# ilia-glushchenko/SimplePathTracer

Measured on AMD Instinct MI355X. Metric: Msamples/s (pixels×spp/s), RTIOW random-sphere scene, 1/2/4/8 MI355X, higher is better.
Workload: dtype f32

## Files before the change

### simplepathtracer_amd/csrc/spt_internal.h

```cpp
#pragma once
#include <hip/hip_runtime.h>
#include <stdint.h>

#include "spt_hip.h"

namespace spt {

struct RowMap {
    uint32_t y0, y1, strip, parts, part;
    uint32_t x0, width;
};

__host__ __device__ inline uint32_t row_of(const RowMap &m, uint32_t lr)
{
    uint32_t blk = lr / m.strip;
    return m.y0 + (blk * m.parts + m.part) * m.strip + (lr - blk * m.strip);
}

__host__ __device__ inline uint32_t rows_owned(const RowMap &m)
{
    if (m.y1 <= m.y0) return 0;
    uint32_t h = m.y1 - m.y0;
    uint32_t period = m.strip * m.parts;
    uint32_t full = h / period, rem = h % period;
// ... 43 lines not shown
inline FastDiv make_fastdiv(uint32_t d)
{
    FastDiv f{d, 0u, 0u};
    if (d <= 1u) return f;
    uint32_t l = 0;
    while ((1ull << l) < d) ++l;
    f.m = (uint32_t)(((1ull << (31 + l)) / d) + 1ull);
    f.s = l - 1u;
    return f;
}
__host__ __device__ inline uint32_t fast_div(uint32_t x, const FastDiv &f)
{
#ifdef __HIP_DEVICE_COMPILE__
    const uint32_t hi = __umulhi(x, f.m);
#else
    const uint32_t hi = (uint32_t)(((uint64_t)x * f.m) >> 32);
#endif
    return f.d <= 1u ? x : hi >> f.s;
}

__host__ __device__ inline uint32_t row_of_fast(const RowMap &m, uint32_t lr, const FastDiv &div_strip)
{
    const uint32_t blk = fast_div(lr, div_strip);
    return m.y0 + (blk * m.parts + m.part) * m.strip + (lr - blk * m.strip);
}

struct DealRule {
    uint64_t below;
    uint32_t q, rem;
};
constexpr DealRule make_deal_rule(uint32_t np)
{
    DealRule r{0ull, 0u, 0u};
    if (np == 0u || np > 64u) return r;
    r.q = 64u / np;
    r.rem = 64u - r.q * np;
    uint32_t start = 0;
    for (uint32_t k = 0; k < np; ++k) {
        if (start > 0u) r.below |= 1ull << (start - 1u);
        start += r.q + (k < r.rem ? 1u : 0u);
    }
    return r;
}
struct DealTable {
    DealRule e[65];
    constexpr DealTable() : e{}
    {
        for (uint32_t np = 0; np <= 64u; ++np) e[np] = make_deal_rule(np);
    }
};
static constexpr DealTable kDealTable{};
__host__ __device__ inline uint32_t deal_start(const DealRule &r, uint32_t rank)
{
    return rank * r.q + (rank < r.rem ? rank : r.rem);
}
__host__ __device__ inline uint32_t deal_count(const DealRule &r, uint32_t rank)
{
    return r.q + (rank < r.rem ? 1u : 0u);
}
__host__ __device__ inline void deal_lane(const DealRule &r, uint32_t lane, uint32_t &rank, uint32_t &tt)
{
#ifdef __HIP_DEVICE_COMPILE__
    rank = __builtin_amdgcn_mbcnt_hi((uint32_t)(r.below >> 32), __builtin_amdgcn_mbcnt_lo((uint32_t)r.below, 0u));
#else
    rank = (uint32_t)__builtin_popcountll(r.below & ((1ull << lane) - 1ull));
#endif
    tt = lane - deal_start(r, rank);
}

__host__ __device__ inline void ts_item(uint32_t q, uint32_t width, uint32_t rows, uint32_t S, const FastDiv &div_band,
                                        const FastDiv &div_tile, uint32_t &sl, uint32_t &lr, uint32_t &col)
{
    const uint32_t band = rows >= 8u ? fast_div(q, div_band) : 0u;
    const uint32_t h = rows - (band << 3) < 8u ? rows - (band << 3) : 8u;
    const uint32_t qb = q - band * 8u * width * S;
    const uint32_t ft = width >> 3, wr = width & 7u;
    const uint32_t ti = h * 8u * S;
    uint32_t e, wt, c0;
    if (h == 8u) {
        const uint32_t t = fast_div(qb, div_tile);
        if (t < ft) {
            e = qb - t * 64u * S;
            sl = e >> 6;
            const uint32_t pix = e & 63u;
            lr = (band << 3) + (pix >> 3);
            col = (t << 3) + (pix & 7u);
            return;
        }
        e = qb - ft * ti;
        wt = wr;
        c0 = ft << 3;
    } else {
        const uint32_t t = qb / ti;
        wt = t < ft ? 8u : wr;
        e = qb - (t < ft ? t : ft) * ti;
        c0 = (t < ft ? t : ft) << 3;
    }
    sl = e / (h * wt);
    const uint32_t pix = e - sl * h * wt;
    const uint32_t row = pix / wt;
    lr = (band << 3) + row;
    col = c0 + (pix - row * wt);
}

__host__ __device__ inline void ts_slot_base(uint32_t lr, uint32_t col, uint32_t width, uint32_t rows, uint32_t S,
                                             uint32_t &q0, uint32_t &step)
{
    const uint32_t band = lr >> 3;
    const uint32_t h = rows - (band << 3) < 8u ? rows - (band << 3) : 8u;
    const uint32_t ft = width >> 3, wr = width & 7u;
    const uint32_t t = col >> 3;
    const uint32_t tc = t < ft ? t : ft;
    const uint32_t wt = t < ft ? 8u : wr;
    q0 = band * 8u * width * S + tc * h * 8u * S + (lr - (band << 3)) * wt + (col - (tc << 3));
    step = h * wt;
}

constexpr uint32_t kCodeSmall = 0x33800000u;
constexpr uint32_t kCodeMax = 2u * (kCodeSmall - 1u);
constexpr uint32_t kCodeSat = 280;
__host__ __device__ inline bool code_layout_fits(uint64_t stride, uint32_t jmax)
// ... 271 lines not shown
```

### simplepathtracer_amd/csrc/spt_kernels.hip

```cpp
#include "spt_path.h"
#include "spt_decode.h"

#include <algorithm>
#include <mutex>

namespace spt {


#ifndef SPT_WAVES_PER_EU
#define SPT_WAVES_PER_EU 0
#endif
#ifndef SPT_NUM_SGPR
#define SPT_NUM_SGPR 96
#endif
#if SPT_WAVES_PER_EU
#define SPT_RENDER_ATTR __attribute__((amdgpu_waves_per_eu(SPT_WAVES_PER_EU, SPT_WAVES_PER_EU)))
#elif SPT_NUM_SGPR
#define SPT_CAP_WAVES (800 / (((SPT_NUM_SGPR - 2 + 15) / 16) * 16 + 16) > 8 ? 8 : 800 / (((SPT_NUM_SGPR - 2 + 15) / 16) * 16 + 16))
#define SPT_RENDER_ATTR __attribute__((amdgpu_num_sgpr(SPT_NUM_SGPR), amdgpu_waves_per_eu(SPT_CAP_WAVES)))
#else
#define SPT_RENDER_ATTR
#endif

#ifndef SPT_LDS_BLOCK
// ... 305 lines not shown
            if (v.y != 0u) {
                const f3 c = decode_sample(a, v.x);
                acc.x = acc.x + c.x;
                acc.y = acc.y + c.y;
                acc.z = acc.z + c.z;
                acc.w = acc.w + 1.f;
            }
        }
    } else {
        alias_accumulate(a, samples, p, W, rows, 0u, rows, S, acc);
    }
    if (!a.last) {
        a.acc[p] = acc;
        if (!a.preview) return;
    }
    const float scale = a.mode == 0 ? 1.f / (float)a.s_done : 1.f / acc.w;
    const float r = acc.x * scale, g = acc.y * scale, b = acc.z * scale;
    if (out_rgba) out_rgba[p] = make_float4(r, g, b, 0.f);
    if (out_rgb8) {
        const uint32_t x = map.x0 + col;
        const uint32_t y = row_of(map, lr);
        const size_t gi = (size_t)3 * ((size_t)(a.height - 1u - y) * a.width + x);
        out_rgb8[gi + 0] = gamma_byte(r);
        out_rgb8[gi + 1] = gamma_byte(g);
        out_rgb8[gi + 2] = gamma_byte(b);
    }
}

#ifndef SPT_SVC_WT
#define SPT_SVC_WT 1
#endif

__device__ __forceinline__ void svc_flush(uint32_t idx, uint32_t cnt, uint32_t lane)
{
    if (cnt == 0u) return;
    kargs_t &k = *kernarg_args();
    asm volatile("s_waitcnt vmcnt(0)" ::: "memory");
    if (!SPT_SVC_WT) {
        __builtin_amdgcn_fence(__ATOMIC_RELEASE, "agent");
        asm volatile("s_waitcnt vmcnt(0)" ::: "memory");
    }
    if (lane == 0) __hip_atomic_fetch_add((gu32 *)(k.svc_done + idx), cnt, __ATOMIC_RELAXED, __HIP_MEMORY_SCOPE_AGENT);
    if (k.svc_trace && lane == 0) atomicMax(k.svc_trace + 4u * idx + 2u, __builtin_amdgcn_s_memrealtime());
}

template <bool TREE, int LEAF, bool LDSN, uint32_t BLOCK, bool BATCH = false, bool GLANE = false, bool SVC = false>
__device__ __forceinline__ void render_body(const RenderArgs &a)
{
    static_assert(!SVC || (!GLANE && !BATCH && (LDSN || SPT_PRIM)),
                  "the render service runs the wave-walk kernel or the LDS lane walk");
    const uint32_t lane = __lane_id();
    const uint32_t rows = SVC ? 0u : a.npix / a.map.width;

    __shared__ uint32_t s_lds[BLOCK];
    __shared__ uint4 s_nodes[LDSN ? 2 * (SVC ? kLdsSvcNodeRecords : kLdsNodeRecords) : 1];
    constexpr bool LDS_BYTES = LDSN && SPT_LANE_WALK && SPT_LANE_BUDGET > 0;
    constexpr bool PRIM = SPT_PRIM && !LDSN && !GLANE;
    constexpr uint32_t PW = kParkWords + (SVC ? 1u : 0u);
    __shared__ uint32_t s_park[PRIM ? (BLOCK / 64u) * PW * 64u : 1];
    uint32_t *const park = s_park + (PRIM ? opaque_v((threadIdx.x >> 6) * PW * 64u + lane) : 0u);
    auto prow = [&](uint32_t r) -> int32_t { return (int32_t)r - (int32_t)lane; };
    __shared__ uint32_t s_rec[SVC ? (BLOCK / 64u) * kSvcRecWords : 1];
    uint32_t *const rec = s_rec + (SVC ? (threadIdx.x >> 6) * kSvcRecWords : 0u);
    if (SVC && lane < kSvcRecWords - kSvcSt) rec[kSvcSt + lane] = 0u;
    if (SVC && !LDSN && blockIdx.x == 0u && (threadIdx.x >> 6) == 0u) {
        svc_forward(lane);
        return;
    }
    uint32_t q_n = 0, q_pos = 0;
    if (LDSN) {
        const uint4 *src = (const uint4 *)a.scene.accel.nodes;
        const uint32_t n4 = 2u * (a.scene.accel.n_nodes + 1u);
        for (uint32_t k = threadIdx.x; k < n4; k += BLOCK) {
            uint4 v = src[k];
            if (LDS_BYTES && (k & 1u)) v.x <<= 5;
            s_nodes[k] = v;
        }
        __syncthreads();
        if (SVC && blockIdx.x == 0u && (threadIdx.x >> 6) == 0u) {
            svc_forward(lane);
            return;
        }
    }
    Path ps;
    ps.phase = PH_IDLE;
    ps.item = ps.bounce = ps.spec = 0;
    ps.st = 0;
    ps.o = ps.d = mk(0.f, 0.f, 0.f);
    ps.slot = 0;
    ps.job = 0;

    uint32_t blk_cur = 0, blk_end = 0;
    uint32_t pend = 0;
    uint32_t rect = 0;
    const uint32_t home = blockIdx.x % a.n_queues;
    uint32_t qi = 0;
    if (SVC)
        pend = svc_reserve(home, lane, 0u);
    else if (lane == 0)
        pend = claim_next(a, home, qi);
    bool exhausted = false;
    uint32_t acc_idx = 0, acc_cnt = 0;
    unsigned long long casts = 0, done = 0, dropped = 0;
    struct {
        unsigned long long iters = 0, cast = 0, shade = 0, refill = 0;
        unsigned long long p_iters = 0, p_nodes = 0, p_spheres = 0, p_branches = 0, p_cast = 0;
        unsigned long long s_rounds[3] = {0, 0, 0};
        unsigned long long t_iters = 0, t_live = 0;
    } dc;
    CastDiag dg;
    Hit hres;
    hres.idx = kMiss;
    hres.best = FLT_MAX;
    hres.t = 0.f;
    uint32_t li = 0, lleaf = kNoSlot, lleaf2 = kNoSlot;
    bool fresh = true;
#if SPT_DIAG
// ... 219 lines not shown
                }
                if (leave) break;
                continue;
            }
            if (exhausted && q_pos == q_n) break;
            continue;
        }
        SPT_STAMP(dc.refill);
#if SPT_DIAG
        const unsigned long long d_n0 = dg.nodes, d_s0 = dg.spheres, d_b0 = dg.branches, d_c0 = dc.cast;
#endif
        constexpr bool RES = SPT_LANE_BUDGET > 0 && (LDSN || GLANE);
        if (!RES) casts += (unsigned long long)__popcll(live);
        ++dc.iters;
        if (SPT_DIAG && exhausted) {
            dc.t_iters += 1;
            dc.t_live += (unsigned long long)__popcll(live);
        }
        const bool act = ps.phase != PH_IDLE;
        bool cdone = true;
        Hit h;
        if constexpr (RES) {
            if (SPT_DUP & 512) {
                Hit h2 = hres;
                h2.best = opaque_v(h2.best);
                uint32_t li2 = opaque_v(li), ll2 = lleaf, ll22 = lleaf2;
                const bool c2 = lane_cast<LEAF, LDS_BYTES>(a.scene.accel, opaque_v3(ps.o), opaque_v3(ps.d), act, dg,
                                    LDSN ? (const uint32_t *)s_nodes : (const uint32_t *)a.scene.accel.nodes, fresh,
                                    (uint32_t)SPT_LANE_BUDGET, h2, li2, ll2, ll22);
                sink_v(h2.idx);
                sink_v(h2.best);
                sink_v(li2);
                sink_v(c2 ? 1u : 0u);
            }
            cdone = lane_cast<LEAF, LDS_BYTES>(a.scene.accel, ps.o, ps.d, act, dg,
                                    LDSN ? (const uint32_t *)s_nodes : (const uint32_t *)a.scene.accel.nodes, fresh,
                                    (uint32_t)SPT_LANE_BUDGET, hres, li, lleaf, lleaf2);
            h = hres;
            casts += (unsigned long long)__popcll(__ballot(act && cdone));
        } else if constexpr (PRIM) {
            bool listed = false;
            if (prim_iter && kernarg_args()->prim.on) {
                if (SPT_DUP & 64) {
                    Hit h2;
                    prim_list_cast(a.scene.accel, opaque_v3(ps.o), opaque_v3(ps.d), act, pxy, h2, dg);
                    sink_v(h2.idx);
                    sink_v(h2.best);
                    sink_v(h2.t);
                }
                listed = prim_list_cast(a.scene.accel, ps.o, ps.d, act, pxy, h, dg);
            }
            if (!listed)
                h = find_closest<TREE, LEAF, LDSN>(a.scene.accel, ps.o, ps.d, act, dg, (const uint32_t *)s_nodes,
                                                   s_lds + (threadIdx.x & ~63u));
            if (SPT_DUP & 1) {
                const f3 o2 = opaque_v3(ps.o), d2 = opaque_v3(ps.d);
                Hit h2;
                bool l2 = false;
                if (prim_iter && kernarg_args()->prim.on) l2 = prim_list_cast(a.scene.accel, o2, d2, act, pxy, h2, dg);
                if (!l2) h2 = find_closest<TREE, LEAF, LDSN>(a.scene.accel, o2, d2, act, dg, (const uint32_t *)s_nodes);
                sink_v(h2.idx);
                sink_v(h2.best);
                sink_v(h2.t);
            }
        } else {
            h = (LDSN && SPT_LANE_WALK)
                    ? find_closest_lane<LEAF>(a.scene.accel, ps.o, ps.d, act, dg, (const uint32_t *)s_nodes)
                : GLANE
                    ? find_closest_lane<LEAF>(a.scene.accel, ps.o, ps.d, act, dg, (const uint32_t *)a.scene.accel.nodes)
                    : find_closest<TREE, LEAF, LDSN>(a.scene.accel, ps.o, ps.d, act, dg, (const uint32_t *)s_nodes);
        }
        SPT_STAMP(dc.cast);
#if SPT_DIAG
        if (prim_iter) {
            dc.p_iters += 1;
            dc.p_nodes += dg.nodes - d_n0;
            dc.p_spheres += dg.spheres - d_s0;
            dc.p_branches += dg.branches - d_b0;
            dc.p_cast += dc.cast - d_c0;
        }
#endif
        shade_step<true, SVC && SPT_SVC_WT>(a, ps, h, act && cdone, done, dropped, s_lds + (threadIdx.x & ~63u),
                                            SPT_DIAG ? dc.s_rounds : nullptr);
        fresh = cdone;
        if (SVC) {
            const bool fin = act && ps.phase == PH_IDLE;
            unsigned long long fm = __ballot(fin);
            while (fm != 0ull) {
                const uint32_t j = __builtin_amdgcn_readlane(ps.job, (int)__builtin_ctzll(fm));
                const unsigned long long m = __ballot(fin && ps.job == j);
                if (j != acc_idx) {
                    svc_flush(acc_idx, acc_cnt, lane);
                    acc_idx = j;
                    acc_cnt = 0;
                }
                acc_cnt += (uint32_t)__popcll(m);
                fm &= ~m;
            }
        }
        if (PRIM && prim_iter) {
            Path own;
            unpark_path<SVC>(park, 0, own);
            __builtin_amdgcn_wave_barrier();
            const unsigned long long lv = __ballot(ps.phase != PH_IDLE);
            if (ps.phase != PH_IDLE) park_path<SVC>(park, prow(lane_rank(lv)), ps);
            ps = own;
            q_n = (uint32_t)__popcll(lv);
            q_pos = 0;
        }
        SPT_STAMP(dc.shade);
    }

    if (SVC) {
        svc_flush(acc_idx, acc_cnt, lane);
        kargs_t &k = *kernarg_args();
        if (lane == 0) __hip_atomic_fetch_add((gu32 *)(k.svc_ctl + kSvcLive), 0xFFFFFFFFu, __ATOMIC_RELAXED, __HIP_MEMORY_SCOPE_AGENT);
    }
#pragma unroll
    for (int o = 32; o > 0; o >>= 1) {
        done += __shfl_xor(done, o);
        dropped += __shfl_xor(dropped, o);
    }
    if (lane == 0) {
        if (casts) atomicAdd(&a.counters[0], casts);
        if (done) atomicAdd(&a.counters[1], done);
        if (dropped) atomicAdd(&a.counters[2], dropped);
    }
#if SPT_DIAG
    if (lane == 0) {
        atomicAdd(&a.counters[4], dc.iters);
        atomicAdd(&a.counters[5], dg.leaves);
        atomicAdd(&a.counters[6], dg.nodes);
        atomicAdd(&a.counters[7], dc.cast);
        atomicAdd(&a.counters[8], dc.shade);
        atomicAdd(&a.counters[9], dc.refill);
// ... 353 lines not shown
```

### simplepathtracer_amd/csrc/spt_path.h

```cpp
#pragma once
#include "spt_device.h"
#include "spt_internal.h"

#include <float.h>

#ifndef SPT_GROUP
#define SPT_GROUP 4
#endif

#ifndef SPT_DIAG
#define SPT_DIAG 0
#endif
#ifndef SPT_LEAF_SPLIT
#define SPT_LEAF_SPLIT 1
#endif
#ifndef SPT_DUP
#define SPT_DUP 0
#endif
#ifndef SPT_SAMPLER_SKIP0
#define SPT_SAMPLER_SKIP0 1
#endif
#ifndef SPT_SAMPLER_EVEN
#define SPT_SAMPLER_EVEN 1
#endif
#ifndef SPT_LEAF_PAIRS
#define SPT_LEAF_PAIRS 2
#endif


#pragma clang fp contract(off)

namespace spt {
namespace {

constexpr uint32_t PH_IDLE = 0, PH_TRACE = 1, PH_DLOOP = 2;

constexpr float kRsq = ((1.0f - 1.5f) / (1.0f + 1.5f)) * ((1.0f - 1.5f) / (1.0f + 1.5f));
static_assert(kRsq == 0x1.47ae16p-5f, "rSq");
constexpr float kAirToGlass = 1.0f / 1.5f;
constexpr float kGlassToAir = 1.5f / 1.0f;

typedef __attribute__((address_space(4))) const float cfloat;
typedef __attribute__((address_space(4))) const uint32_t cuint;

__device__ __forceinline__ float4 ld_uniform(cfloat *p, uint32_t i)
{
    return make_float4(p[4 * i + 0], p[4 * i + 1], p[4 * i + 2], p[4 * i + 3]);
}

__device__ __forceinline__ float max_raw(float a, float b)
{
    float r;
    asm("v_max_f32 %0, %1, %2" : "=v"(r) : "v"(a), "v"(b));
    return r;
}
__device__ __forceinline__ float min_raw(float a, float b)
{
    float r;
    asm("v_min_f32 %0, %1, %2" : "=v"(r) : "v"(a), "v"(b));
    return r;
}
__device__ __forceinline__ float max3_raw(float a, float b, float c)
{
    float r;
    asm("v_max3_f32 %0, %1, %2, %3" : "=v"(r) : "v"(a), "v"(b), "v"(c));
    return r;
}
__device__ __forceinline__ float min3_raw(float a, float b, float c)
{
    float r;
    asm("v_min3_f32 %0, %1, %2, %3" : "=v"(r) : "v"(a), "v"(b), "v"(c));
    return r;
}

__device__ __forceinline__ uint32_t lane_rank(unsigned long long mask)
{
// ... 685 lines not shown
            continue;
        }
        if (SPT_DIAG) dg.live += 1;
        auto visit = [&]() {
            const uint4 *rec = BYTES ? (const uint4 *)((const char *)lnodes + i) : ln + 2 * i;
            const uint4 ra = rec[0], rb = rec[1];
            const uint32_t nskip = rb.x, nslot = rb.y;
            const float ax = __builtin_fmaf(__uint_as_float(ra.x), irx, qlx);
            const float bx = __builtin_fmaf(__uint_as_float(ra.w), irx, qhx);
            const float ay = __builtin_fmaf(__uint_as_float(ra.y), iry, qly);
            const float by = __builtin_fmaf(__uint_as_float(rb.z), iry, qhy);
            const float az = __builtin_fmaf(__uint_as_float(ra.z), irz, qlz);
            const float bz = __builtin_fmaf(__uint_as_float(rb.w), irz, qhz);
            const float tn = max3_raw(__builtin_fminf(ax, bx), __builtin_fminf(ay, by),
                                      max_raw(__builtin_fminf(az, bz), neta));
            const float tf = min3_raw(__builtin_fmaxf(ax, bx), __builtin_fmaxf(ay, by),
                                      min_raw(__builtin_fmaxf(az, bz), sbl));
            const bool hit = (tn <= tf) | nocull;
            const bool is_leaf = nslot != kNoSlot;
            if (hit && is_leaf) {
                leaf2 = leaf;
                leaf = nslot;
            }
            i = (hit && !is_leaf) ? i + (BYTES ? 32u : 1u) : nskip;
        };
#pragma unroll
        for (int k = 0; k < SPT_LANE_STEPS; ++k) {
            const bool w = i < n && leaf2 == kNoSlot;
            if (SPT_DIAG) dg.nodes += (unsigned long long)__popcll(__ballot(w));
            if (w) visit();
        }
    }
    return !(i < n || leaf != kNoSlot);
}

template <int LEAF>
__device__ __forceinline__ Hit find_closest_lane(const AccelView &ac, const f3 &o, const f3 &d, bool active,
                                                 CastDiag &dg, const uint32_t *lnodes)
{
    Hit h;
    uint32_t i, leaf, leaf2;
    (void)lane_cast<LEAF>(ac, o, d, active, dg, lnodes, true, 0xFFFFFFFFu, h, i, leaf, leaf2);
    return h;
}

struct Path {
    uint32_t phase, item, bounce, spec;
    uint64_t st;
    f3 o, d;
    uint32_t slot;
    uint32_t job;
};

__device__ __forceinline__ f3 coop_ball_vector(uint64_t &st, bool need, uint32_t *lds, unsigned long long *rounds = nullptr)
{
    const uint32_t lane = __lane_id();
    const uint64_t st0 = st;
    f3 r;
    uint32_t jacc = 0;
    unsigned long long pend;
    uint32_t jb;
    const unsigned long long needm = __ballot(need);
    if (SPT_SAMPLER_SKIP0 && __popcll(needm) <= 32) {
        r = mk(0.f, 0.f, 0.f);
        pend = needm;
        jb = 0;
    } else {
        uint64_t t = st0;
        r.x = uniform(t, -0.5f, 0.5f);
        r.y = uniform(t, -0.5f, 0.5f);
        r.z = uniform(t, -0.5f, 0.5f);
        pend = __ballot(need && lensq(r) < 0.25f);
        jb = 1;
    }
    const uint32_t s_lo = (uint32_t)st0, s_hi = (uint32_t)(st0 >> 32);
    if (SPT_DIAG && rounds) rounds[0] += 1;
#if SPT_DIAG
    const unsigned long long t_in = __builtin_amdgcn_s_memtime();
#endif
#if SPT_SAMPLER_EVEN
    if (jb != 0u) jacc = __builtin_amdgcn_inverse_ballot_w64(pend) ? 1u : 0u;
    while (pend != 0ull) {
        if (SPT_DIAG && rounds) rounds[1] += 1;
        const DealRule dr = kDealTable.e[__popcll(pend)];
        const bool is_p = __builtin_amdgcn_inverse_ballot_w64(pend);
        const uint32_t rank = lane_rank(pend);
        if (is_p) lds[rank] = (jacc << 6) | lane;
        uint32_t pidx, tt;
        deal_lane(dr, lane, pidx, tt);
        const uint32_t w = lds[pidx];
        const uint32_t src = w & 63u;
        const uint32_t h_lo = (uint32_t)__shfl((int)s_lo, (int)src), h_hi = (uint32_t)__shfl((int)s_hi, (int)src);
        uint64_t b = (((uint64_t)h_hi << 32) | h_lo) + (uint64_t)(3u * ((w >> 6) + tt)) * kGamma;
        f3 c;
        c.x = uniform(b, -0.5f, 0.5f);
        c.y = uniform(b, -0.5f, 0.5f);
        c.z = uniform(b, -0.5f, 0.5f);
        const unsigned long long acc = __ballot(!(lensq(c) < 0.25f));
        const uint32_t start = deal_start(dr, rank), cnt = deal_count(dr, rank);
        const unsigned long long seg = acc >> (start & 63u);
        const uint32_t tstar = seg != 0ull ? (uint32_t)__builtin_ctzll(seg) : 64u;
        const bool found = is_p && tstar < cnt;
        const uint32_t from = found ? start + tstar : lane;
        const float rx = __shfl(c.x, (int)from), ry = __shfl(c.y, (int)from), rz = __shfl(c.z, (int)from);
        if (found) r = mk(rx, ry, rz);
        if (is_p) jacc += tstar < cnt ? tstar : cnt;
        pend = __ballot(is_p && !found);
    }
#else
    while (pend != 0ull) {
        if (SPT_DIAG && rounds) rounds[1] += 1;
        const uint32_t np = (uint32_t)__popcll(pend);
        uint32_t lg = np <= 4u ? 4u : (uint32_t)__builtin_clz(np - 1u) - 26u;
        lg = lg > 4u ? 4u : lg;
        const bool is_p = __builtin_amdgcn_inverse_ballot_w64(pend);
        const uint32_t rank = lane_rank(pend);
        if (is_p) lds[rank] = lane;
        const uint32_t pidx = lane >> lg, tt = lane & ((1u << lg) - 1u);
        const bool valid = pidx < np;
        const uint32_t src = lds[valid ? pidx : 0u];
        const uint32_t h_lo = (uint32_t)__shfl((int)s_lo, (int)src), h_hi = (uint32_t)__shfl((int)s_hi, (int)src);
        uint64_t b = (((uint64_t)h_hi << 32) | h_lo) + (uint64_t)(3u * (jb + tt)) * kGamma;
        f3 c;
        c.x = uniform(b, -0.5f, 0.5f);
        c.y = uniform(b, -0.5f, 0.5f);
        c.z = uniform(b, -0.5f, 0.5f);
        const unsigned long long acc = __ballot(valid && !(lensq(c) < 0.25f));
        const uint32_t seg = is_p ? (uint32_t)(acc >> (rank << lg)) & ((1u << (1u << lg)) - 1u) : 0u;
        const bool found = seg != 0u;
        const uint32_t tstar = found ? (uint32_t)__builtin_ctz(seg) : 0u;
        const uint32_t from = found ? (rank << lg) + tstar : lane;
        const float rx = __shfl(c.x, (int)from), ry = __shfl(c.y, (int)from), rz = __shfl(c.z, (int)from);
        if (found) {
            r = mk(rx, ry, rz);
            jacc = jb + tstar;
        }
        pend = __ballot(is_p && !found);
        jb += 1u << lg;
    }
#endif
    if (need) st = st0 + (uint64_t)(3u * (jacc + 1u)) * kGamma;
#if SPT_DIAG
    if (rounds) rounds[2] += __builtin_amdgcn_s_memtime() - t_in;
#endif
    return r;
}

typedef __attribute__((address_space(4))) const RenderArgs kargs_t;
__device__ __forceinline__ kargs_t *kernarg_args()
{
    uint32_t z;
    asm volatile("s_mov_b32 %0, 0" : "=s"(z));
    typedef __attribute__((address_space(4))) const char kchar;
    return (kargs_t *)((kchar *)__builtin_amdgcn_kernarg_segment_ptr() + z);
}

__device__ __forceinline__ bool prim_list_cast(const AccelView &ac, const f3 &o, const f3 &d, bool active, uint32_t pxy,
                                               Hit &h, CastDiag &dg)
{
    kargs_t &k = *kernarg_args();
    const float ddev = lensq(d) - 1.0f;
    if (__ballot(active && !(ddev <= 1e-6f && ddev >= -1e-6f && lensq(o) <= 1e30f)) != 0ull) return false;
    h.idx = kMiss;
    h.best = FLT_MAX;
    h.t = 0.f;
    const unsigned long long live = __ballot(active);
    if (live == 0ull) return true;
    const uint32_t bw = k.prim.bw;
    const uint32_t x = pxy & 0xFFFFu, y = pxy >> 16;
    const float dod = dot(o, d);
    cfloat *slots = (cfloat *)ac.slots;
    cuint *ids = (cuint *)k.prim.slots;
    if (SPT_DIAG) dg.live_now = (uint32_t)__popcll(live);
    auto test_run = [&](uint2 e) {
        for (uint32_t i = e.x; i < e.x + e.y; i += 4u) {
            uint32_t s[4];
            float4 sp[4];
#pragma unroll
            for (int q = 0; q < 4; ++q) s[q] = ids[i + q];
#pragma unroll
            for (int q = 0; q < 4; ++q) sp[q] = ld_uniform(slots, s[q]);
            float tcv[4], hv[4];
            bool pass[4];
#pragma unroll
            for (int q = 0; q < 4; ++q) pass[q] = ray_sphere(sp[q], o, d, tcv[q], hv[q]);
            if (SPT_DIAG) dg.lane_tests += 4ull * dg.live_now;
#pragma unroll
            for (int q = 0; q < 4; ++q) {
                const unsigned long long pm = __ballot(pass[q]);
                if (SPT_DIAG) {
                    dg.spheres += 1;
                    dg.branches += pm != 0ull ? 1 : 0;
                }
                if (pm != 0ull) update_member(pm, tcv[q], hv[q], ac.orig, s[q], o, d, dod, h, dg);
// ... 49 lines not shown
            nd = reflect(d2, n2);
    } else {
        nd = reflect(d, nrm);
    }
    ps.d = nd;
}

template <bool WT = false>
__device__ __forceinline__ void finish_step(uint32_t mode, uint32_t *samples, Path &ps, bool fin, bool spec_event,
                                            bool refr_event, bool sky, uint32_t word, unsigned long long &done,
                                            unsigned long long &dropped)
{
    bool counted = true;
    if (spec_event) {
        const uint32_t k = ps.spec & 0xFFFFu;
        if (mode == 1u && k < kTaskPasses && refr_event) ps.spec |= 1u << (16u + k);
        ++ps.spec;
        if (mode == 1u && k + 1u >= kTaskPasses) {
            fin = true;
            counted = false;
            word = kZeroWord;
            ++dropped;
        } else if (k + 1u > kSpecularCap) {
            fin = true;
            word = kZeroWord;
        }
    }
    if (fin) {
        typedef __attribute__((address_space(1))) uint32_t gu32_t;
        typedef __attribute__((address_space(1))) unsigned long long gu64_t;
        if (mode == 0u) {
            if (WT)
                __hip_atomic_store((gu32_t *)(samples + ps.item), word, __ATOMIC_RELAXED, __HIP_MEMORY_SCOPE_AGENT);
            else
                samples[ps.item] = word;
        } else {
            const uint32_t key =
                counted ? 1u + (((ps.spec & 0xFFFFu) << 11) | (sky ? 1u << 10 : 0u) | ((ps.spec >> 16) & 0x3FFu)) : 0u;
            if (WT)
                __hip_atomic_store((gu64_t *)(samples + (size_t)2 * ps.item), (unsigned long long)word | ((unsigned long long)key << 32),
                                   __ATOMIC_RELAXED, __HIP_MEMORY_SCOPE_AGENT);
            else
                *(uint2 *)(samples + (size_t)2 * ps.item) = make_uint2(word, key);
        }
        ps.phase = PH_IDLE;
        ps.d = mk(0.f, 0.f, 0.f);
        ++done;
    }
}

template <bool KARG, bool WT, bool SAMPLER>
__device__ __forceinline__ void shade_step_body(const RenderArgs &a, Path &ps, const Hit &h, bool act,
                                                unsigned long long &done, unsigned long long &dropped, uint32_t *lds,
                                                unsigned long long *diag_rounds)
{
    const float4 *__restrict__ hit = a.scene.accel.slots;
    const float4 *__restrict__ shade = a.scene.shade;
    const uint32_t *__restrict__ mat = a.scene.mat;
    uint32_t *samples = a.samples;
    uint32_t mode = a.mode;
    uint32_t bounces = a.bounces, code_stride = a.scene.code_stride, code_jmax = a.scene.code_jmax;
    if constexpr (KARG) {
        kargs_t &k = *kernarg_args();
        hit = k.scene.accel.slots;
        shade = k.scene.shade;
        mat = k.scene.mat;
        samples = k.samples;
        mode = k.mode;
        bounces = k.bounces;
        code_stride = k.scene.code_stride;
        code_jmax = k.scene.code_jmax;
    }
    const uint32_t idx = h.idx;
    bool fin = false;
    uint32_t word = kZeroWord;
    const bool dl = ps.phase == PH_DLOOP;
    uint32_t m = SPT_SKYBOX_ID;
    if (act && idx != kMiss) m = mat[idx];
    bool scatter = false, refr = false;
    if (!act) {
    } else if (dl) {
        --ps.bounce;
        const bool end = ps.bounce == 0u || idx == kMiss;
        if (end) {
            const uint32_t j = min(bounces - ps.bounce - 1u, code_jmax);
            word = code_word(diffuse_code(j, ps.slot, code_stride));
            fin = true;
        }
        scatter = !end;
        refr = false;
    } else {
        scatter = m == SPT_DIFFUSE_ID || m == SPT_REFLECTIVE_ID;
        refr = m == SPT_REFRACTIVE_ID;
        if (!scatter && !refr) {
            word = __float_as_uint(ps.d.y + 1.f);
            fin = true;
        }
    }
    bool spec_event = false;
    const f3 rv_coop = SAMPLER ? coop_ball_vector(ps.st, scatter, lds, diag_rounds) : opaque_v3(mk(0.1f, 0.2f, 0.3f));
    if ((SPT_DUP & 2) && SAMPLER) {
        uint64_t st2 = opaque_v(ps.st);
        const f3 r2 = coop_ball_vector(st2, opaque_v(scatter ? 1u : 0u) != 0u, lds);
        sink_v(r2.x);
        sink_v(r2.y);
        sink_v(r2.z);
        sink_v(st2);
    }
    if (scatter) {
        const float4 cs = hit[idx];
        const f3 C = mk(cs.x, cs.y, cs.z);
        ps.o = contact(ps.o, ps.d, h.t);
        const f3 nrm = normalize(sub(ps.o, C));
        f3 rv = rv_coop;
        f3 base;
        if (dl) {
            base = add(ps.o, nrm);
        } else if (m == SPT_DIFFUSE_ID) {
            ps.slot = idx;
            base = nrm;
            ps.phase = PH_DLOOP;
        } else {
            base = reflect(ps.d, nrm);
            rv = mul(rv, shade[idx].w);
            spec_event = true;
        }
        ps.d = normalize(add(base, rv));
    }
    if (refr) {
        ps.o = contact(ps.o, ps.d, h.t);
        if (SPT_DUP & 256) {
            Path p2 = ps;
            p2.o = opaque_v3(p2.o);
            refract_event(hit, p2, idx);
            sink_v(p2.d.x);
            sink_v(p2.o.x);
            sink_v(p2.st);
        }
        refract_event(hit, ps, idx);
        spec_event = true;
    }
    finish_step<WT>(mode, samples, ps, fin, spec_event, refr, !dl, word, done, dropped);
}
template <bool KARG = false, bool WT = false>
__device__ __forceinline__ void shade_step(const RenderArgs &a, Path &ps, const Hit &h, bool act,
                                           unsigned long long &done, unsigned long long &dropped, uint32_t *lds,
                                           unsigned long long *diag_rounds = nullptr)
{
    if (SPT_DUP & 128) {
        Path p2 = ps;
        p2.o = opaque_v3(p2.o);
        p2.d = opaque_v3(p2.d);
        Hit h2 = h;
        h2.t = opaque_v(h2.t);
        unsigned long long d2 = 0, x2 = 0;
        shade_step_body<KARG, WT, false>(a, p2, h2, act, d2, x2, lds, nullptr);
        sink_v(p2.o.x);
        sink_v(p2.d.x);
        sink_v(p2.st);
    }
    shade_step_body<KARG, WT, true>(a, ps, h, act, done, dropped, lds, diag_rounds);
}



__device__ __forceinline__ void start_path(const RenderArgs &a, uint32_t mine, uint32_t rows, const Recip &rw,
                                           const Recip &rh, const f3 &eye, Path &ps, uint32_t *pxy = nullptr)
{
    uint32_t sl, lr, cx;
    ts_item(mine, a.map.width, rows, a.spp_batch, a.div_band, a.div_tile, sl, lr, cx);
    const uint32_t s = a.s0 + sl;
    ps.item = mine;
    const uint32_t x = a.map.x0 + cx;
    const uint32_t y = a.map.parts == 1u ? a.map.y0 + lr : row_of_fast(a.map, lr, a.div_strip);
    if (pxy) *pxy = (y << 16) | x;
    ps.st = fmix64(a.seed_key ^ (((uint64_t)(y * a.width + x) << 32) | (uint64_t)s));
    const float un = (float)y + uniform(ps.st, -1.f, 1.f);
    const float vn = (float)x + uniform(ps.st, -1.f, 1.f);
    float u = div_core(un, rw), v = div_core(vn, rh);
    if (__builtin_expect(!(div_operand_ok(un) && div_operand_ok(vn)), 0)) {
        u = un / (float)a.width;
        v = vn / (float)a.height;
    }
    const float vx = -1.f + 2.f * v, vy = -1.f + 2.f * u;
    const float *m = a.cam.view;
    ps.d = normalize(mk((m[0] * vx + m[1] * vy) + (m[2] * 1.f + m[3] * 0.f),
                        (m[4] * vx + m[5] * vy) + (m[6] * 1.f + m[7] * 0.f),
                        (m[8] * vx + m[9] * vy) + (m[10] * 1.f + m[11] * 0.f)));
    ps.o = eye;
    ps.phase = PH_TRACE;
    ps.bounce = a.bounces;
    ps.spec = 0;
}

__device__ __forceinline__ void start_path_kernarg(uint32_t mine, uint32_t rows, Path &ps, uint32_t *pxy = nullptr)
{
    kargs_t &k = *kernarg_args();
    RenderArgs a;
    a.map = RowMap{k.map.y0, k.map.y1, k.map.strip, k.map.parts, k.map.part, k.map.x0, k.map.width};
    a.width = k.width;
    a.height = k.height;
    a.bounces = k.bounces;
    a.npix = k.npix;
    a.n_items = k.n_items;
    a.spp_batch = k.spp_batch;
    a.s0 = k.s0;
    a.seed_key = k.seed_key;
    a.div_band = FastDiv{k.div_band.d, k.div_band.m, k.div_band.s};
    a.div_tile = FastDiv{k.div_tile.d, k.div_tile.m, k.div_tile.s};
    a.div_strip = FastDiv{k.div_strip.d, k.div_strip.m, k.div_strip.s};
#pragma unroll
    for (int q = 0; q < 12; ++q) a.cam.view[q] = k.cam.view[q];
    start_path(a, mine, rows, recip((float)a.width), recip((float)a.height),
               mk(k.cam.eye[0], k.cam.eye[1], k.cam.eye[2]), ps, pxy);
// ... 66 lines not shown
```

### simplepathtracer_amd/csrc/spt_trace.hip

```cpp
#include "spt_query.h"
#include "spt_decode.h"

namespace spt {

namespace {

constexpr uint32_t kTraceLaunchRays = 1u << 28;

template <bool TREE, int LEAF, int WALK, uint32_t BLOCK>
__device__ __forceinline__ void trace_body(const TraceArgs &a)
{
    constexpr bool AHEAD = WALK != kWalkLds;
    __shared__ uint32_t s_lds[BLOCK];
    const AccelView &ac = a.scene.accel;
    const uint32_t *const nodes = lds_node_table<WALK, BLOCK>(ac);
    RenderArgs ra;
    ra.scene = a.scene;
    ra.bounces = a.bounces;
    ra.mode = 0u;
    ra.samples = (uint32_t *)a.rgba;
    uint32_t *const lds = s_lds + (threadIdx.x & ~63u);

    const uint32_t lane = __lane_id();
    const uint32_t wave = __builtin_amdgcn_readfirstlane(blockIdx.x * (BLOCK / 64u) + (threadIdx.x >> 6));
    const uint32_t n_waves = gridDim.x * (BLOCK / 64u);
    const uint32_t runs = (a.n + 63u) >> 6;
    uint32_t run = wave, q_n = 0, q_pos = 0;
    f3 qo = mk(0.f, 0.f, 0.f), qd = mk(0.f, 0.f, 0.f);
    uint32_t qs_lo = 0, qs_hi = 0;
    auto load_run = [&]() {
        q_n = run < runs ? min(64u, a.n - (run << 6)) : 0u;
        q_pos = 0;
        if (AHEAD && lane < q_n) {
            const uint32_t i = (run << 6) + lane;
            const float4 o4 = a.o[i], d4 = a.d[i];
            const uint64_t st = a.st[i];
            qo = mk(o4.x, o4.y, o4.z);
            qd = mk(d4.x, d4.y, d4.z);
            qs_lo = (uint32_t)st;
            qs_hi = (uint32_t)(st >> 32);
        }
    };
    load_run();

    Path ps;
    ps.phase = PH_IDLE;
    ps.item = ps.bounce = ps.spec = 0;
    ps.st = 0;
    ps.o = ps.d = mk(0.f, 0.f, 0.f);
    ps.slot = 0;
    ps.job = 0;
    uint32_t casts = 0;
    unsigned long long done = 0, dropped = 0;
    CastDiag dg;

    for (;;) {
        const unsigned long long need = __ballot(ps.phase == PH_IDLE);
        if (need != 0ull && q_n != 0u) {
            const uint32_t take = min((uint32_t)__popcll(need), q_n - q_pos);
            const uint32_t rank = lane_rank(need);
            const bool get = __builtin_amdgcn_inverse_ballot_w64(need) && rank < take;
            const int from = (int)(get ? q_pos + rank : lane);
            f3 o = mk(0.f, 0.f, 0.f), d = o;
            uint64_t st = 0;
            if (AHEAD) {
                o = mk(__shfl(qo.x, from), __shfl(qo.y, from), __shfl(qo.z, from));
                d = mk(__shfl(qd.x, from), __shfl(qd.y, from), __shfl(qd.z, from));
                st = ((uint64_t)(uint32_t)__shfl((int)qs_hi, from) << 32) | (uint32_t)__shfl((int)qs_lo, from);
            }
            if (get) {
                const uint32_t i = (run << 6) + (uint32_t)from;
                if (!AHEAD) {
                    const float4 o4 = a.o[i], d4 = a.d[i];
                    st = a.st[i];
                    o = mk(o4.x, o4.y, o4.z);
                    d = mk(d4.x, d4.y, d4.z);
                }
                ps.o = o;
                ps.d = d;
                ps.st = st;
                ps.item = 4u * i;
                ps.phase = PH_TRACE;
                ps.bounce = a.bounces;
                ps.spec = 0;
                casts = 0;
            }
            q_pos += take;
            if (q_pos == q_n) {
                run += n_waves;
                load_run();
            }
        }
        const unsigned long long live = __ballot(ps.phase != PH_IDLE);
        if (live == 0ull) {
            if (q_n == 0u) break;
            continue;
        }
        const bool act = ps.phase != PH_IDLE;
        const Hit h = query_cast<TREE, LEAF, WALK>(ac, ps.o, ps.d, act, dg, nodes, lds);
        casts += act ? 1u : 0u;
        shade_step(ra, ps, h, act, done, dropped, lds);
        if (act && ps.phase == PH_IDLE && a.info) {
            const uint32_t ev = ps.spec & 0xFFFFu;
            uint32_t *rec = a.info + (ps.item >> 1);
            rec[0] = casts;
            rec[1] = ev | (ev > kSpecularCap ? 0x80000000u : 0u);
        }
    }
}

constexpr uint32_t kTraceBlock = 256, kTraceLdsBlock = 1024;

}

template <bool TREE, int LEAF>
__global__ __launch_bounds__(kTraceBlock) __attribute__((amdgpu_waves_per_eu(6))) void trace_kernel(TraceArgs a)
{
    trace_body<TREE, LEAF, kWalkWave, kTraceBlock>(a);
}
__global__ __launch_bounds__(kTraceBlock) void trace_kernel_glane(TraceArgs a)
{
    trace_body<true, (int)kClusterSlots, kWalkGlane, kTraceBlock>(a);
}
__global__ __launch_bounds__(kTraceLdsBlock) __attribute__((amdgpu_waves_per_eu(2 * kTraceLdsBlock / 256))) void trace_kernel_lds(TraceArgs a)
{
    trace_body<true, (int)kClusterSlots, kWalkLds, kTraceLdsBlock>(a);
}

__global__ __launch_bounds__(256) void trace_decode_kernel(FoldArgs f, float4 *rgba, uint32_t n)
{
    const uint32_t i = blockIdx.x * 256u + threadIdx.x;
    if (i >= n) return;
    const f3 c = decode_sample(f, f.samples[4u * i]);
    rgba[i] = make_float4(c.x, c.y, c.z, 0.f);
}

hipError_t launch_trace(const TraceArgs &all, const FoldArgs &fa, hipStream_t s)
{
    void (*const kernels[5])(TraceArgs) = {trace_kernel_lds, trace_kernel_glane, trace_kernel<true, (int)kClusterSlots>,
                                           trace_kernel<false, (int)kFlatLeafSlots>, trace_kernel<false, (int)kClusterSlots>};
    for (uint64_t r0 = 0; r0 < all.n; r0 += kTraceLaunchRays) {
        TraceArgs a = all;
        a.n = (uint32_t)std::min<uint64_t>(kTraceLaunchRays, all.n - r0);
        a.o += r0;
        a.d += r0;
        a.st += r0;
        a.rgba += r0;
        if (a.info) a.info += 2u * r0;
        hipError_t e = launch_query(a.scene.accel, kernels, kTraceBlock, kTraceLdsBlock, (a.n + 63u) / 64u, s, a);
        if (e != hipSuccess) return e;
        FoldArgs f = fa;
        f.samples = (const uint32_t *)a.rgba;
        hipLaunchKernelGGL(trace_decode_kernel, dim3((a.n + 255u) / 256u), dim3(256), 0, s, f, a.rgba, a.n);
        if ((e = hipGetLastError()) != hipSuccess) return e;
// ... 6 lines not shown
```

### simplepathtracer_amd/csrc/spt_wavefront.hip

```cpp
#include "spt_path.h"

#include <algorithm>
#include <mutex>

namespace spt {

namespace {

constexpr uint32_t kWfBlock = 256;
constexpr uint32_t kWfWaves = kWfBlock / 64;

struct WfQueue {
    float4 *o, *d;
    uint4 *m;
};

struct WfArgs {
    RenderArgs ra;
    WfQueue q;
    uint32_t *state;
    uint32_t qcap;
};

__device__ __forceinline__ void load_ray(const WfQueue &q, uint32_t i, Path &ps)
{
    const float4 o = q.o[i], d = q.d[i];
    const uint4 m = q.m[i];
    ps.o = mk(o.x, o.y, o.z);
    ps.slot = __float_as_uint(o.w);
    ps.d = mk(d.x, d.y, d.z);
    ps.item = __float_as_uint(d.w);
    ps.st = (uint64_t)m.x | ((uint64_t)m.y << 32);
    ps.bounce = m.z;
    ps.phase = m.w & 3u;
    ps.spec = m.w >> 2;
}

__device__ __forceinline__ void store_ray(const WfQueue &q, uint32_t i, const Path &ps)
{
    q.o[i] = make_float4(ps.o.x, ps.o.y, ps.o.z, __uint_as_float(ps.slot));
    q.d[i] = make_float4(ps.d.x, ps.d.y, ps.d.z, __uint_as_float(ps.item));
    q.m[i] = make_uint4((uint32_t)ps.st, (uint32_t)(ps.st >> 32), ps.bounce, ps.phase | (ps.spec << 2));
}

template <bool TREE, int LEAF, bool GLANE>
__global__ __launch_bounds__(kWfBlock) void wf_render(WfArgs w)
{
    __shared__ float4 s_o[kWfBlock], s_d[kWfBlock];
    __shared__ uint4 s_m[kWfBlock];
    __shared__ float2 s_h[kWfBlock];
    __shared__ uint32_t s_lds[kWfBlock];
    __shared__ uint32_t s_cnt[kWfWaves][kWfCats + 1];
    __shared__ uint32_t s_claim;

    typedef __attribute__((address_space(1))) uint32_t gu32;
    const RenderArgs &a = w.ra;
    const uint32_t tid = threadIdx.x, wave = tid >> 6, lane = __lane_id();
    const uint32_t rows = a.npix / a.map.width;
    const Recip rw = recip((float)a.width), rh = recip((float)a.height);
    const f3 eye = mk(a.cam.eye[0], a.cam.eye[1], a.cam.eye[2]);
    const size_t q0 = (size_t)blockIdx.x * w.qcap;
    const WfQueue q{w.q.o + q0, w.q.d + q0, w.q.m + q0};
    uint32_t len = 0;
    unsigned long long cast = 0, finished = 0, done = 0, dropped = 0;
    for (;;) {
        if (tid == 0) s_claim = __hip_atomic_fetch_add((gu32 *)w.state, w.qcap - len, __ATOMIC_RELAXED, __HIP_MEMORY_SCOPE_AGENT);
        __syncthreads();
        const uint32_t first = s_claim;
        const uint32_t got = first < a.n_items ? min(w.qcap - len, a.n_items - first) : 0u;
        const uint32_t n = len + got;
        if (n == 0u) break;
        uint32_t wp = 0;
        for (uint32_t base = 0; base < n; base += kWfBlock) {
            const uint32_t i = base + tid;
            const uint32_t live = min(n - base, kWfBlock);
            const bool act = i < n;
            Path ps;
            ps.phase = PH_IDLE;
            ps.item = ps.bounce = ps.spec = ps.slot = 0;
            ps.st = 0;
            ps.o = ps.d = mk(0.f, 0.f, 0.f);
            if (act) {
                if (i < len) {
                    load_ray(q, i, ps);
                } else {
                    start_path(a, first + (i - len), rows, rw, rh, eye, ps);
                    ps.slot = 0;
                }
            }
            CastDiag dg;
            const Hit h = GLANE ? find_closest_lane<LEAF>(a.scene.accel, ps.o, ps.d, act, dg, (const uint32_t *)a.scene.accel.nodes)
                                : find_closest<TREE, LEAF>(a.scene.accel, ps.o, ps.d, act, dg);
            uint32_t cat = kWfCats;
            if (act) {
                cat = 0u;
                if (ps.phase == PH_DLOOP) {
                    cat = 4u;
                } else if (h.idx != kMiss) {
                    const uint32_t mt = a.scene.mat[h.idx];
                    cat = mt == SPT_DIFFUSE_ID ? 1u : mt == SPT_REFLECTIVE_ID ? 2u : mt == SPT_REFRACTIVE_ID ? 3u : 0u;
                }
            }
            uint32_t rank = 0;
#pragma unroll
            for (uint32_t c = 0; c < kWfCats; ++c) {
                const unsigned long long m = __ballot(cat == c);
                if (lane == 0) s_cnt[wave][c] = (uint32_t)__popcll(m);
                if (cat == c) rank = lane_rank(m);
            }
            __syncthreads();
            if (act) {
                uint32_t pos = rank;
#pragma unroll
                for (uint32_t c = 0; c < kWfCats; ++c)
#pragma unroll
                    for (uint32_t v = 0; v < kWfWaves; ++v)
                        if (c < cat || (c == cat && v < wave)) pos += s_cnt[v][c];
                s_o[pos] = make_float4(ps.o.x, ps.o.y, ps.o.z, __uint_as_float(ps.slot));
                s_d[pos] = make_float4(ps.d.x, ps.d.y, ps.d.z, __uint_as_float(ps.item));
                s_m[pos] = make_uint4((uint32_t)ps.st, (uint32_t)(ps.st >> 32), ps.bounce, ps.phase | (ps.spec << 2));
                s_h[pos] = make_float2(h.t, __uint_as_float(h.idx));
            }
            __syncthreads();
            const bool act2 = tid < live;
            Hit hh;
            hh.best = 0.f;
            hh.t = 0.f;
            hh.idx = kMiss;
            if (act2) {
                const float4 o = s_o[tid], d = s_d[tid];
                const uint4 m = s_m[tid];
                const float2 t = s_h[tid];
                ps.o = mk(o.x, o.y, o.z);
                ps.slot = __float_as_uint(o.w);
                ps.d = mk(d.x, d.y, d.z);
                ps.item = __float_as_uint(d.w);
                ps.st = (uint64_t)m.x | ((uint64_t)m.y << 32);
                ps.bounce = m.z;
                ps.phase = m.w & 3u;
                ps.spec = m.w >> 2;
                hh.t = t.x;
                hh.idx = __float_as_uint(t.y);
            } else {
                ps.phase = PH_IDLE;
            }
            shade_step(a, ps, hh, act2, done, dropped, s_lds + wave * 64u);
            const bool alive = act2 && ps.phase != PH_IDLE;
            const unsigned long long am = __ballot(alive);
            if (lane == 0) s_cnt[wave][kWfCats] = (uint32_t)__popcll(am);
            __syncthreads();
            uint32_t at = wp + lane_rank(am), tot = 0;
#pragma unroll
            for (uint32_t v = 0; v < kWfWaves; ++v) {
                const uint32_t k = s_cnt[v][kWfCats];
                if (v < wave) at += k;
                tot += k;
            }
            if (alive) store_ray(q, at, ps);
            wp += tot;
            __syncthreads();
        }
        cast += n;
        finished += n - wp;
        len = wp;
    }
    (void)done;
    if (tid == 0) {
        atomicAdd(&a.counters[0], cast);
        atomicAdd(&a.counters[1], finished);
    }
    if (dropped) atomicAdd(&a.counters[2], dropped);
}

template <bool TREE, int LEAF, bool GLANE>
uint32_t resident_blocks(int dev)
{
    static std::mutex mu;
    static int cached[64];
    std::lock_guard<std::mutex> lk(mu);
    if (dev < 0 || dev >= 64) return 0;
    if (cached[dev] == 0) {
        int per_cu = 0, cus = 0;
        if (hipOccupancyMaxActiveBlocksPerMultiprocessor(&per_cu, wf_render<TREE, LEAF, GLANE>, kWfBlock, 0) != hipSuccess ||
            hipDeviceGetAttribute(&cus, hipDeviceAttributeMultiprocessorCount, dev) != hipSuccess)
            return 0;
        cached[dev] = std::max(per_cu, 0) * std::max(cus, 0);
        if (cached[dev] == 0) cached[dev] = -1;
    }
    return cached[dev] > 0 ? (uint32_t)cached[dev] : 0u;
}

template <bool TREE, int LEAF, bool GLANE>
hipError_t launch(const WavefrontBuffers &b, const RenderArgs &a, hipStream_t s)
{
    int dev = 0;
    hipError_t e = hipGetDevice(&dev);
    if (e != hipSuccess) return e;
    const uint32_t resident = resident_blocks<TREE, LEAF, GLANE>(dev);
    if (resident == 0) return hipErrorInvalidConfiguration;
// ... 33 lines not shown
```

Measured before the change: 25260.

## Table sampler steps in LDS and shrink per-wave sampler scratch to bytes

Rewrites the cooperative rejection sampler for random-in-unit-ball. It now keeps a running RNG state that advances by a table of precomputed gamma step offsets held in LDS, instead of tracking a draw counter and multiplying at the end. Lane ids are stored as bytes, so per-wave LDS scratch shrinks from 64 words to 16 when the node table is in LDS. The change also drops the non-even deal path and uses 24-bit multiplies in deal_start. The aim is to cut 64-bit multiplies and LDS footprint, which may help occupancy. In exchange it adds a table fill and a barrier in some kernels, and the wavefront kernel reads the table without a visible sync after filling it.

```diff
diff --git a/simplepathtracer_amd/csrc/spt_internal.h b/simplepathtracer_amd/csrc/spt_internal.h
--- a/simplepathtracer_amd/csrc/spt_internal.h
+++ b/simplepathtracer_amd/csrc/spt_internal.h
@@ -119,7 +119,11 @@
 static constexpr DealTable kDealTable{};
 __host__ __device__ inline uint32_t deal_start(const DealRule &r, uint32_t rank)
 {
+#ifdef __HIP_DEVICE_COMPILE__
+    return __umul24(rank, r.q) + (rank < r.rem ? rank : r.rem);
+#else
     return rank * r.q + (rank < r.rem ? rank : r.rem);
+#endif
 }
 __host__ __device__ inline uint32_t deal_count(const DealRule &r, uint32_t rank)
 {
@@ -134,6 +138,10 @@
 #endif
     tt = lane - deal_start(r, rank);
 }
+
+constexpr uint64_t kSamplerGamma = 0x9E3779B97F4A7C15ull;
+constexpr uint32_t kSamplerSteps = 65;
+__host__ __device__ constexpr uint64_t sampler_step(uint32_t t) { return (uint64_t)(3u * t) * kSamplerGamma; }
 
 __host__ __device__ inline void ts_item(uint32_t q, uint32_t width, uint32_t rows, uint32_t S, const FastDiv &div_band,
                                         const FastDiv &div_tile, uint32_t &sl, uint32_t &lr, uint32_t &col)
diff --git a/simplepathtracer_amd/csrc/spt_kernels.hip b/simplepathtracer_amd/csrc/spt_kernels.hip
--- a/simplepathtracer_amd/csrc/spt_kernels.hip
+++ b/simplepathtracer_amd/csrc/spt_kernels.hip
@@ -381,7 +381,8 @@
     const uint32_t lane = __lane_id();
     const uint32_t rows = SVC ? 0u : a.npix / a.map.width;
 
-    __shared__ uint32_t s_lds[BLOCK];
+    constexpr uint32_t LW = LDSN ? kSamplerLdsWords : 64u;
+    __shared__ uint32_t s_lds[(BLOCK / 64u) * LW];
     __shared__ uint4 s_nodes[LDSN ? 2 * (SVC ? kLdsSvcNodeRecords : kLdsNodeRecords) : 1];
     constexpr bool LDS_BYTES = LDSN && SPT_LANE_WALK && SPT_LANE_BUDGET > 0;
     constexpr bool PRIM = SPT_PRIM && !LDSN && !GLANE;
@@ -392,6 +393,9 @@
     __shared__ uint32_t s_rec[SVC ? (BLOCK / 64u) * kSvcRecWords : 1];
     uint32_t *const rec = s_rec + (SVC ? (threadIdx.x >> 6) * kSvcRecWords : 0u);
     if (SVC && lane < kSvcRecWords - kSvcSt) rec[kSvcSt + lane] = 0u;
+    __shared__ uint64_t s_steps[kSamplerSteps];
+    fill_sampler_steps(s_steps);
+    if (!LDSN) __syncthreads();
     if (SVC && !LDSN && blockIdx.x == 0u && (threadIdx.x >> 6) == 0u) {
         svc_forward(lane);
         return;
@@ -717,7 +721,7 @@
             }
             if (!listed)
                 h = find_closest<TREE, LEAF, LDSN>(a.scene.accel, ps.o, ps.d, act, dg, (const uint32_t *)s_nodes,
-                                                   s_lds + (threadIdx.x & ~63u));
+                                                   s_lds + (threadIdx.x >> 6) * LW);
             if (SPT_DUP & 1) {
                 const f3 o2 = opaque_v3(ps.o), d2 = opaque_v3(ps.d);
                 Hit h2;
@@ -745,7 +749,7 @@
             dc.p_cast += dc.cast - d_c0;
         }
 #endif
-        shade_step<true, SVC && SPT_SVC_WT>(a, ps, h, act && cdone, done, dropped, s_lds + (threadIdx.x & ~63u),
+        shade_step<true, SVC && SPT_SVC_WT>(a, ps, h, act && cdone, done, dropped, s_lds + (threadIdx.x >> 6) * LW, s_steps,
                                             SPT_DIAG ? dc.s_rounds : nullptr);
         fresh = cdone;
         if (SVC) {
diff --git a/simplepathtracer_amd/csrc/spt_path.h b/simplepathtracer_amd/csrc/spt_path.h
--- a/simplepathtracer_amd/csrc/spt_path.h
+++ b/simplepathtracer_amd/csrc/spt_path.h
@@ -19,9 +19,6 @@
 #endif
 #ifndef SPT_SAMPLER_SKIP0
 #define SPT_SAMPLER_SKIP0 1
-#endif
-#ifndef SPT_SAMPLER_EVEN
-#define SPT_SAMPLER_EVEN 1
 #endif
 #ifndef SPT_LEAF_PAIRS
 #define SPT_LEAF_PAIRS 2
@@ -813,46 +810,50 @@
     uint32_t job;
 };
 
-__device__ __forceinline__ f3 coop_ball_vector(uint64_t &st, bool need, uint32_t *lds, unsigned long long *rounds = nullptr)
-{
+constexpr uint32_t kSamplerLdsWords = 16;
+__device__ __forceinline__ void fill_sampler_steps(uint64_t *steps)
+{
+    if (threadIdx.x < kSamplerSteps) steps[threadIdx.x] = sampler_step(threadIdx.x);
+}
+__device__ __forceinline__ f3 coop_ball_vector(uint64_t &st, bool need, uint32_t *lds, const uint64_t *steps,
+                                               unsigned long long *rounds = nullptr)
+{
+    static_assert(sampler_step(1) == 3ull * kGamma, "the table steps by three draws");
     const uint32_t lane = __lane_id();
-    const uint64_t st0 = st;
+    uint8_t *const ids = (uint8_t *)lds;
+    uint64_t S = st;
     f3 r;
-    uint32_t jacc = 0;
     unsigned long long pend;
-    uint32_t jb;
     const unsigned long long needm = __ballot(need);
     if (SPT_SAMPLER_SKIP0 && __popcll(needm) <= 32) {
         r = mk(0.f, 0.f, 0.f);
         pend = needm;
-        jb = 0;
     } else {
-        uint64_t t = st0;
+        uint64_t t = S;
         r.x = uniform(t, -0.5f, 0.5f);
         r.y = uniform(t, -0.5f, 0.5f);
         r.z = uniform(t, -0.5f, 0.5f);
         pend = __ballot(need && lensq(r) < 0.25f);
-        jb = 1;
-    }
-    const uint32_t s_lo = (uint32_t)st0, s_hi = (uint32_t)(st0 >> 32);
+        if (need) S = t;
+    }
     if (SPT_DIAG && rounds) rounds[0] += 1;
 #if SPT_DIAG
     const unsigned long long t_in = __builtin_amdgcn_s_memtime();
 #endif
-#if SPT_SAMPLER_EVEN
-    if (jb != 0u) jacc = __builtin_amdgcn_inverse_ballot_w64(pend) ? 1u : 0u;
     while (pend != 0ull) {
         if (SPT_DIAG && rounds) rounds[1] += 1;
         const DealRule dr = kDealTable.e[__popcll(pend)];
         const bool is_p = __builtin_amdgcn_inverse_ballot_w64(pend);
         const uint32_t rank = lane_rank(pend);
-        if (is_p) lds[rank] = (jacc << 6) | lane;
+        if (is_p) ids[rank] = (uint8_t)lane;
         uint32_t pidx, tt;
         deal_lane(dr, lane, pidx, tt);
-        const uint32_t w = lds[pidx];
-        const uint32_t src = w & 63u;
-        const uint32_t h_lo = (uint32_t)__shfl((int)s_lo, (int)src), h_hi = (uint32_t)__shfl((int)s_hi, (int)src);
-        uint64_t b = (((uint64_t)h_hi << 32) | h_lo) + (uint64_t)(3u * ((w >> 6) + tt)) * kGamma;
+        const uint32_t src = ids[pidx];
+        const uint32_t h_lo = (uint32_t)__shfl((int)(uint32_t)S, (int)src);
+        const uint32_t h_hi = (uint32_t)__shfl((int)(uint32_t)(S >> 32), (int)src);
+        typedef uint32_t u32x2 __attribute__((ext_vector_type(2)));
+        const u32x2 hv = {h_lo, h_hi};
+        uint64_t b = __builtin_bit_cast(uint64_t, hv) + steps[tt];
         f3 c;
         c.x = uniform(b, -0.5f, 0.5f);
         c.y = uniform(b, -0.5f, 0.5f);
@@ -865,42 +866,11 @@
         const uint32_t from = found ? start + tstar : lane;
         const float rx = __shfl(c.x, (int)from), ry = __shfl(c.y, (int)from), rz = __shfl(c.z, (int)from);
         if (found) r = mk(rx, ry, rz);
-        if (is_p) jacc += tstar < cnt ? tstar : cnt;
-        pend = __ballot(is_p && !found);
-    }
-#else
-    while (pend != 0ull) {
-        if (SPT_DIAG && rounds) rounds[1] += 1;
-        const uint32_t np = (uint32_t)__popcll(pend);
-        uint32_t lg = np <= 4u ? 4u : (uint32_t)__builtin_clz(np - 1u) - 26u;
-        lg = lg > 4u ? 4u : lg;
-        const bool is_p = __builtin_amdgcn_inverse_ballot_w64(pend);
-        const uint32_t rank = lane_rank(pend);
-        if (is_p) lds[rank] = lane;
-        const uint32_t pidx = lane >> lg, tt = lane & ((1u << lg) - 1u);
-        const bool valid = pidx < np;
-        const uint32_t src = lds[valid ? pidx : 0u];
-        const uint32_t h_lo = (uint32_t)__shfl((int)s_lo, (int)src), h_hi = (uint32_t)__shfl((int)s_hi, (int)src);
-        uint64_t b = (((uint64_t)h_hi << 32) | h_lo) + (uint64_t)(3u * (jb + tt)) * kGamma;
-        f3 c;
-        c.x = uniform(b, -0.5f, 0.5f);
-        c.y = uniform(b, -0.5f, 0.5f);
-        c.z = uniform(b, -0.5f, 0.5f);
-        const unsigned long long acc = __ballot(valid && !(lensq(c) < 0.25f));
-        const uint32_t seg = is_p ? (uint32_t)(acc >> (rank << lg)) & ((1u << (1u << lg)) - 1u) : 0u;
-        const bool found = seg != 0u;
-        const uint32_t tstar = found ? (uint32_t)__builtin_ctz(seg) : 0u;
-        const uint32_t from = found ? (rank << lg) + tstar : lane;
-        const float rx = __shfl(c.x, (int)from), ry = __shfl(c.y, (int)from), rz = __shfl(c.z, (int)from);
-        if (found) {
-            r = mk(rx, ry, rz);
-            jacc = jb + tstar;
-        }
-        pend = __ballot(is_p && !found);
-        jb += 1u << lg;
-    }
-#endif
-    if (need) st = st0 + (uint64_t)(3u * (jacc + 1u)) * kGamma;
+        const uint32_t adv = is_p ? (tstar < cnt ? tstar + 1u : cnt) : 0u;
+        S += steps[adv];
+        pend &= ~__ballot(tstar < cnt);
+    }
+    st = S;
 #if SPT_DIAG
     if (rounds) rounds[2] += __builtin_amdgcn_s_memtime() - t_in;
 #endif
@@ -1056,7 +1026,7 @@
 template <bool KARG, bool WT, bool SAMPLER>
 __device__ __forceinline__ void shade_step_body(const RenderArgs &a, Path &ps, const Hit &h, bool act,
                                                 unsigned long long &done, unsigned long long &dropped, uint32_t *lds,
-                                                unsigned long long *diag_rounds)
+                                                const uint64_t *steps, unsigned long long *diag_rounds)
 {
     const float4 *__restrict__ hit = a.scene.accel.slots;
     const float4 *__restrict__ shade = a.scene.shade;
@@ -1102,10 +1072,10 @@
         }
     }
     bool spec_event = false;
-    const f3 rv_coop = SAMPLER ? coop_ball_vector(ps.st, scatter, lds, diag_rounds) : opaque_v3(mk(0.1f, 0.2f, 0.3f));
+    const f3 rv_coop = SAMPLER ? coop_ball_vector(ps.st, scatter, lds, steps, diag_rounds) : opaque_v3(mk(0.1f, 0.2f, 0.3f));
     if ((SPT_DUP & 2) && SAMPLER) {
         uint64_t st2 = opaque_v(ps.st);
-        const f3 r2 = coop_ball_vector(st2, opaque_v(scatter ? 1u : 0u) != 0u, lds);
+        const f3 r2 = coop_ball_vector(st2, opaque_v(scatter ? 1u : 0u) != 0u, lds, steps);
         sink_v(r2.x);
         sink_v(r2.y);
         sink_v(r2.z);
@@ -1149,7 +1119,7 @@
 template <bool KARG = false, bool WT = false>
 __device__ __forceinline__ void shade_step(const RenderArgs &a, Path &ps, const Hit &h, bool act,
                                            unsigned long long &done, unsigned long long &dropped, uint32_t *lds,
-                                           unsigned long long *diag_rounds = nullptr)
+                                           const uint64_t *steps, unsigned long long *diag_rounds = nullptr)
 {
     if (SPT_DUP & 128) {
         Path p2 = ps;
@@ -1158,12 +1128,12 @@
         Hit h2 = h;
         h2.t = opaque_v(h2.t);
         unsigned long long d2 = 0, x2 = 0;
-        shade_step_body<KARG, WT, false>(a, p2, h2, act, d2, x2, lds, nullptr);
+        shade_step_body<KARG, WT, false>(a, p2, h2, act, d2, x2, lds, steps, nullptr);
         sink_v(p2.o.x);
         sink_v(p2.d.x);
         sink_v(p2.st);
     }
-    shade_step_body<KARG, WT, true>(a, ps, h, act, done, dropped, lds, diag_rounds);
+    shade_step_body<KARG, WT, true>(a, ps, h, act, done, dropped, lds, steps, diag_rounds);
 }
 
 
diff --git a/simplepathtracer_amd/csrc/spt_trace.hip b/simplepathtracer_amd/csrc/spt_trace.hip
--- a/simplepathtracer_amd/csrc/spt_trace.hip
+++ b/simplepathtracer_amd/csrc/spt_trace.hip
@@ -11,7 +11,11 @@
 __device__ __forceinline__ void trace_body(const TraceArgs &a)
 {
     constexpr bool AHEAD = WALK != kWalkLds;
-    __shared__ uint32_t s_lds[BLOCK];
+    constexpr uint32_t LW = WALK == kWalkLds ? kSamplerLdsWords : 64u;
+    __shared__ uint32_t s_lds[(BLOCK / 64u) * LW];
+    __shared__ uint64_t s_steps[kSamplerSteps];
+    fill_sampler_steps(s_steps);
+    if (WALK != kWalkLds) __syncthreads();
     const AccelView &ac = a.scene.accel;
     const uint32_t *const nodes = lds_node_table<WALK, BLOCK>(ac);
     RenderArgs ra;
@@ -19,7 +23,7 @@
     ra.bounces = a.bounces;
     ra.mode = 0u;
     ra.samples = (uint32_t *)a.rgba;
-    uint32_t *const lds = s_lds + (threadIdx.x & ~63u);
+    uint32_t *const lds = s_lds + (threadIdx.x >> 6) * LW;
 
     const uint32_t lane = __lane_id();
     const uint32_t wave = __builtin_amdgcn_readfirstlane(blockIdx.x * (BLOCK / 64u) + (threadIdx.x >> 6));
@@ -99,7 +103,7 @@
         const bool act = ps.phase != PH_IDLE;
         const Hit h = query_cast<TREE, LEAF, WALK>(ac, ps.o, ps.d, act, dg, nodes, lds);
         casts += act ? 1u : 0u;
-        shade_step(ra, ps, h, act, done, dropped, lds);
+        shade_step(ra, ps, h, act, done, dropped, lds, s_steps);
         if (act && ps.phase == PH_IDLE && a.info) {
             const uint32_t ev = ps.spec & 0xFFFFu;
             uint32_t *rec = a.info + (ps.item >> 1);
diff --git a/simplepathtracer_amd/csrc/spt_wavefront.hip b/simplepathtracer_amd/csrc/spt_wavefront.hip
--- a/simplepathtracer_amd/csrc/spt_wavefront.hip
+++ b/simplepathtracer_amd/csrc/spt_wavefront.hip
@@ -52,6 +52,8 @@
     __shared__ uint32_t s_lds[kWfBlock];
     __shared__ uint32_t s_cnt[kWfWaves][kWfCats + 1];
     __shared__ uint32_t s_claim;
+    __shared__ uint64_t s_steps[kSamplerSteps];
+    fill_sampler_steps(s_steps);
 
     typedef __attribute__((address_space(1))) uint32_t gu32;
     const RenderArgs &a = w.ra;
@@ -144,7 +146,7 @@
             } else {
                 ps.phase = PH_IDLE;
             }
-            shade_step(a, ps, hh, act2, done, dropped, s_lds + wave * 64u);
+            shade_step(a, ps, hh, act2, done, dropped, s_lds + wave * 64u, s_steps);
             const bool alive = act2 && ps.phase != PH_IDLE;
             const unsigned long long am = __ballot(alive);
             if (lane == 0) s_cnt[wave][kWfCats] = (uint32_t)__popcll(am);
```

After: 25480, median of 6. No clear change (+0.9%).
